# nithinp7/Pies

Hardware: AMD Instinct MI355X
Metric: substeps/sec @100k particles (PBD distance+tet-strain, 20 iterations) (higher is better)
Workload: dtype f32; 1 GPU; BASELINE configs[1]: 20x20x250 lattice beam, 100000 particles, 649156 distance + 539334 tet-strain constraints, PBD, 20 iterations, 1 substep/tick, collisions off, one body per GPU; schedule=layered, parallelism=replicas x1

## Files before the change

### include/pies_hip.h

```cpp
#ifndef PIES_HIP_H
#define PIES_HIP_H

#include <stdint.h>

#ifdef __cplusplus
extern "C" {
#endif

#define PIES_ABI_VERSION 4

typedef struct pies_solver pies_solver_t;

typedef struct pies_options {
  float fixedTimestepSize;
  uint32_t timeSubsteps;
  uint32_t iterations;
  uint32_t collisionStabilizationIterations;
  float collisionThresholdDistance;
  float collisionThickness;
  float gravity;
  float damping;
  float friction;
  float staticFrictionThreshold;
  float floorHeight;
// ... 17 lines not shown
  PIES_DISTANCE = 1,
  PIES_TET = 2,
  PIES_VOLUME = 3,
  PIES_BEND = 4,
  PIES_SHAPE = 5,
  PIES_GOAL = 6,
  PIES_TRIANGLES = 7,
  PIES_LINES = 8,
  PIES_NODES = 9,
  PIES_SYSTEM_NNZ = 10,
  PIES_REST_SETS = 11,
  PIES_ROW_STENCILS = 12,
  PIES_PD_TILES = 13,
  PIES_PD_TILE_RECORDS = 14,
  PIES_PD_CG_SINGLE = 15,
  PIES_PD_WINDOW_ENTRIES = 16,
  PIES_PD_WINDOW_HALO = 17,
  PIES_NODE_PAIRS = 18,
  PIES_NODES_RENUMBERED = 19,
  PIES_NODE_CONTACTS = 20,
  PIES_SKINS = 21,
  PIES_SKIN_VERTICES = 22,
  PIES_LAYER_REST_SETS = 23,
  PIES_LAYER_MAX_TILES = 24
};

enum { PIES_SCHEDULE_EXACT = 0, PIES_SCHEDULE_COLOURED = 1, PIES_SCHEDULE_LAYERED = 2 };
#define PIES_SCHEDULE_DEFAULT PIES_SCHEDULE_LAYERED

enum {
  PIES_FLAG_RELEASE_HINGE = 0,
  PIES_FLAG_NODE_COLLISIONS = 1,
  PIES_FLAG_TRIANGLE_COLLISIONS = 2,
  PIES_FLAG_REFERENCE_COLLISION_ORDER = 3,
  PIES_FLAG_COLLISION_ORDER = 4,
  PIES_FLAG_RENUMBER_NODES = 5,
  PIES_FLAG_PD_NODE_CONTACTS = 6
};
enum { PIES_COLLISION_ORDER_REFERENCE = 0, PIES_COLLISION_ORDER_GROUPS = 1, PIES_COLLISION_ORDER_PAIRS = 2 };

enum { PIES_NODE_POSITION = 0, PIES_NODE_PREV_POSITION = 1, PIES_NODE_VELOCITY = 2, PIES_NODE_RADIUS = 3, PIES_NODE_INV_MASS = 4 };

#define PIES_DEVICE_NONE (-1)
int pies_create(const pies_options_t* options, int device, pies_solver_t** out);
int pies_destroy(pies_solver_t* s);
int pies_clear(pies_solver_t* s);
const char* pies_last_error(const pies_solver_t* s);
// ... 106 lines not shown
```

### pies_amd/capi.py

```python
import ctypes as C
import os

import numpy as np

HERE = os.path.dirname(os.path.abspath(__file__))
LIB_PATH = os.environ.get("PIES_LIB") or os.path.join(HERE, "lib", "libpies_hip.so")

OK, ERR_INVALID, ERR_HIP, ERR_STATE, ERR_UNSUPPORTED = range(5)
PBD, PD = 0, 1
POSITION, DISTANCE, TET, VOLUME, BEND, SHAPE, GOAL, TRIANGLES, LINES, NODES = range(10)
SCHEDULE_EXACT, SCHEDULE_COLOURED, SCHEDULE_LAYERED = 0, 1, 2
SCHEDULE_DEFAULT = SCHEDULE_LAYERED
DEVICE_NONE = -1
FLAG_RELEASE_HINGE, FLAG_NODE_COLLISIONS, FLAG_TRIANGLE_COLLISIONS, FLAG_REFERENCE_COLLISION_ORDER, FLAG_COLLISION_ORDER = 0, 1, 2, 3, 4
FLAG_RENUMBER_NODES = 5
FLAG_PD_NODE_CONTACTS = 6
COLLISION_ORDER_REFERENCE, COLLISION_ORDER_GROUPS, COLLISION_ORDER_PAIRS = 0, 1, 2
NODE_POSITION, NODE_PREV_POSITION, NODE_VELOCITY, NODE_RADIUS, NODE_INV_MASS = range(5)
KERNEL_NAMES = ["predict", "position", "distance", "tet", "bend", "floor", "velocity", "hash", "collide",
                "pd_predict", "pd_local_distance", "pd_local_tet", "pd_local_volume", "pd_rhs", "pd_spmv", "pd_cg_update",
                "pd_velocity", "wave", "layer"]
KERNEL_PREDICT, KERNEL_POSITION, KERNEL_DISTANCE, KERNEL_TET, KERNEL_BEND, KERNEL_FLOOR, KERNEL_VELOCITY = range(7)
KERNEL_COUNT = 19
SYSTEM_NNZ = 10
REST_SETS = 11
ROW_STENCILS = 12
PD_TILES = 13
PD_TILE_RECORDS = 14
PD_CG_SINGLE = 15
PD_WINDOW_ENTRIES, PD_WINDOW_HALO = 16, 17
NODE_PAIRS = 18
NODES_RENUMBERED = 19
NODE_CONTACTS = 20
SKINS, SKIN_VERTICES = 21, 22
LAYER_REST_SETS = 23
LAYER_MAX_TILES = 24
LAYER_REST_MAX_SETS = 64

SYMBOLS = [
    "pies_create", "pies_destroy", "pies_clear", "pies_last_error", "pies_abi_version", "pies_default_options",
    "pies_get_options", "pies_add_nodes", "pies_add_nodes_ex", "pies_add_position_constraints",
    "pies_add_distance_constraints", "pies_add_tet_constraints", "pies_add_volume_constraints",
    "pies_add_bend_constraints", "pies_add_triangles", "pies_create_tet_box", "pies_create_box", "pies_create_sheet",
    "pies_create_bend_sheet", "pies_set_flag", "pies_set_schedule", "pies_finalize", "pies_tick", "pies_tick_async",
    "pies_synchronize", "pies_failed", "pies_count", "pies_read_nodes", "pies_write_nodes", "pies_get_ids",
    "pies_get_rest", "pies_get_order", "pies_get_batches", "pies_profile_substep", "pies_launch_counts",
    "pies_set_pcg", "pies_get_pcg_stats", "pies_collision_pairs", "pies_add_shape_constraint",
    "pies_add_goal_constraint", "pies_set_goal_transform", "pies_add_fixed_regions", "pies_update_fixed_regions",
    "pies_add_linked_regions", "pies_create_shape_matching_box", "pies_create_shape_matching_sheet", "pies_get_group",
    "pies_get_tri_contacts", "pies_tick_begin", "pies_export_acquire", "pies_export_release",
    "pies_read_positions_strided", "pies_set_pcg_retry", "pies_get_pcg_health", "pies_profile_in_situ",
    "pies_collision_stats", "pies_get_collision_health", "pies_set_collision_rounds", "pies_set_solver", "pies_debug_pair_state", "pies_set_tuning",
    "pies_get_pd_tile_plan", "pies_get_tri_grid_stats", "pies_set_rest", "pies_get_collision_fallbacks",
    "pies_add_node_pair_constraints", "pies_get_node_order", "pies_get_node_contacts",
    "pies_add_skin", "pies_get_skin_binding", "pies_read_skin", "pies_export_acquire_skin",
    "pies_voxelize_tri_mesh", "pies_add_tri_mesh_volume",
    "pies_layer_rest_pack", "pies_layer_rest_unpack", "pies_layer_rest_usable",
]

# ... 567 lines not shown
```

### pies_amd/csrc/capi.cpp

```cpp
#include <algorithm>
#include <cmath>
#include <cstdio>
#include <cstdlib>
#include <cstring>

#include "capi_internal.h"
#include "layer_rest.h"

#include <numeric>

using namespace pies;

extern "C" {

int pies_abi_version(void) { return PIES_ABI_VERSION; }

void pies_default_options(pies_options_t* o) {
  if (!o) return;
  o->fixedTimestepSize = 0.012f;
  o->timeSubsteps = 1;
  o->iterations = 4;
  o->collisionStabilizationIterations = 4;
  o->collisionThresholdDistance = 0.1f;
  o->collisionThickness = 0.05f;
// ... 694 lines not shown
    case PIES_BEND: *out = (uint32_t)s->h_bend.size(); break;
    case PIES_NODE_PAIRS: *out = (uint32_t)s->h_nodePair.size(); break;
    case PIES_SHAPE: *out = (uint32_t)s->h_shape.size(); break;
    case PIES_GOAL: *out = (uint32_t)s->h_goal.size(); break;
    case PIES_TRIANGLES: *out = (uint32_t)(s->h_triangles.size() / 3); break;
    case PIES_LINES: *out = (uint32_t)s->h_lines.size(); break;
    case PIES_NODES: *out = s->nodeCount(); break;
    case PIES_SYSTEM_NNZ: *out = s->pd_nnz; break;
    case PIES_REST_SETS: *out = s->pdLocalPacked && s->dev.d_pairDictIndex ? s->dev.pairDictSets : 0u; break;
    case PIES_ROW_STENCILS: *out = s->dev.pd.cg.rowStencil ? s->dev.pdRowStencils : 0u; break;
    case PIES_PD_TILES: *out = s->dev.pd.tiles.ntiles; break;
    case PIES_PD_TILE_RECORDS: *out = s->dev.pd.tiles.ntiles ? s->pdTileRecords : 0u; break;
    case PIES_PD_CG_SINGLE: *out = s->opt.solver == PIES_SOLVER_PD && pd_single_cg(s) ? 1u : 0u; break;
    case PIES_PD_WINDOW_ENTRIES: *out = s->dev.pd.cg.wRows ? s->pdWindowEntries : 0u; break;
    case PIES_PD_WINDOW_HALO: *out = s->dev.pd.cg.wRows ? s->pdWindowHalo : 0u; break;
    case PIES_NODES_RENUMBERED: *out = s->nodeOrder.active() ? 1u : 0u; break;
    case PIES_LAYER_REST_SETS: *out = s->layer.active ? s->layer.restSets : 0u; break;
    case PIES_LAYER_MAX_TILES: {
      *out = 0;
      if (s->layer.active)
        for (int ph = 0; ph < 4; ++ph) *out = std::max<uint32_t>(*out, (uint32_t)s->layer.tiles[ph].size());
      break;
    }
    case PIES_SKINS: *out = (uint32_t)s->h_skins.size(); break;
    case PIES_SKIN_VERTICES: {
      *out = 0;
      for (const HostSkin& k : s->h_skins) *out += k.vertexCount();
      break;
    }
    case PIES_NODE_CONTACTS: {
      *out = 0;
      if (s->device != PIES_DEVICE_NONE && s->dev.ncActive && s->dev.nd.n)
        if (int rc = nc_download(const_cast<pies_solver*>(s), nullptr, out)) return rc;
      break;
    }
    default: return PIES_ERR_INVALID;
  }
  return PIES_OK;
}

int pies_read_nodes(pies_solver_t* s, int what, float* out, uint32_t n) {
  if (!s || (!out && n)) return PIES_ERR_INVALID;
  if (n != s->nodeCount()) return fail(s, PIES_ERR_INVALID, "pies_read_nodes: n does not match the node count");
  if (s->device != PIES_DEVICE_NONE && what >= PIES_NODE_POSITION && what <= PIES_NODE_VELOCITY) {
    HIP_TRY(s, hipSetDevice(s->device));
    if (int rc = download_nodes(s, 1u << what)) return rc;
// ... 164 lines not shown
```

### pies_amd/csrc/dev_math.h

```cpp
#pragma once
#include <hip/hip_runtime.h>

namespace pies {

#define PIES_DEV __device__ __forceinline__

#ifdef PIES_BOUNDS
static __device__ unsigned int g_pies_bounds[2];
PIES_DEV bool pies_bounds_note(bool ok, unsigned int site) {
  if (!ok) {
    atomicCAS(&g_pies_bounds[0], 0u, site);
    atomicAdd(&g_pies_bounds[1], 1u);
  }
  return ok;
}
#define PIES_IN_BOUNDS(cond, site) (::pies::pies_bounds_note((cond), (site)))
#define PIES_CLAMP_INDEX(i, n) ((i) < (n) ? (i) : 0u)
#define PIES_BOUNDS_REPORT(name)                                                                                     \
  extern "C" int pies_exp_bounds_##name(unsigned int* out) {                                                         \
    unsigned int zero[2] = {0u, 0u};                                                                                 \
    if (hipMemcpyFromSymbol(out, HIP_SYMBOL(::pies::g_pies_bounds), sizeof(zero)) != hipSuccess) return 1;           \
    return hipMemcpyToSymbol(HIP_SYMBOL(::pies::g_pies_bounds), zero, sizeof(zero)) == hipSuccess ? 0 : 1;           \
  }
#else
#define PIES_IN_BOUNDS(cond, site) (true)
#define PIES_CLAMP_INDEX(i, n) (i)
#define PIES_BOUNDS_REPORT(name)
#endif

PIES_DEV uint32_t xcd_block(uint32_t bid, uint32_t nwg) {
  const uint32_t q = nwg >> 3, r = nwg & 7u, x = bid & 7u;
  return (x < r ? x * (q + 1u) : r * (q + 1u) + (x - r) * q) + (bid >> 3);
}

#ifndef PIES_SVD_MAX_SWEEPS
#define PIES_SVD_MAX_SWEEPS 8
#endif
constexpr int kSvdMaxSweeps = PIES_SVD_MAX_SWEEPS;
constexpr float kSvdTol = 4.76837158203125e-07f;
constexpr float kSvdTol2 = kSvdTol * kSvdTol;
constexpr float kSvdTiny = 1.0e-18f;
constexpr float kSvdTiny2 = 1.0e-36f;

struct Svd3 {
  float b[3][3];
  float v[3][3];
  float s[3];
  float rs[3];
};

// ... 131 lines not shown
    const float c00 = fmaf(m11, m22, -(s12 * s12)), c11 = fmaf(m00, m22, -(s02 * s02)), c22 = fmaf(m00, m11, -(s01 * s01));
    const float c01 = fmaf(s02, s12, -(s01 * m22)), c02 = fmaf(s01, s12, -(s02 * m11)), c12 = fmaf(s01, s02, -(s12 * m00));
    const float a0 = fabsf(c00), a1 = fabsf(c11), a2 = fabsf(c22);
    const bool k0 = a0 >= a1 && a0 >= a2, k1 = !k0 && a1 >= a2;
    const float v0 = k0 ? c00 : (k1 ? c01 : c02), v1 = k0 ? c01 : (k1 ? c11 : c12), v2 = k0 ? c02 : (k1 ? c12 : c22);
    const float n2 = fmaf(v2, v2, fmaf(v1, v1, v0 * v0));
    const bool okn = n2 > kSvdTiny2;
    const float in = rsqrt_nr(okn ? n2 : 1.0f);
    const float nx = okn ? v0 * in : 0.0f, ny = okn ? v1 * in : 0.0f, nz = okn ? v2 * in : 1.0f;
    const float sg = __builtin_copysignf(1.0f, nz);
    const float aa = -recip12(fabsf(nz) + 1.0f) * sg;
    const float bb = (nx * ny) * aa;
    const float V[3][3] = {{fmaf(sg * nx, nx * aa, 1.0f), sg * bb, -(sg * nx)}, {bb, fmaf(ny, ny * aa, sg), -ny}, {nx, ny, nz}};
#pragma unroll
    for (int i = 0; i < 3; ++i)
#pragma unroll
      for (int k = 0; k < 3; ++k) {
        d.v[i][k] = V[i][k];
        d.b[i][k] = fmaf(A[2][k], V[i][2], fmaf(A[1][k], V[i][1], A[0][k] * V[i][0]));
      }
    (void)jacobi_pair<0, 1>(d);
    jacobi_polish(d);
  } else {
#pragma unroll
    for (int i = 0; i < 3; ++i)
#pragma unroll
      for (int k = 0; k < 3; ++k) {
        d.b[i][k] = A[i][k];
        d.v[i][k] = (i == k) ? 1.0f : 0.0f;
      }
    if (n01) jacobi_rotate<0, 1>(d, s00, s11, s01);
    else if (n02) jacobi_rotate<0, 2>(d, s00, s22, s02);
    else if (n12) jacobi_rotate<1, 2>(d, s11, s22, s12);
  }
  float n0 = s00, n1 = s11, n2 = s22;
  if (cnt != 0) {
    bool clean = false;
    for (int sweep = 0; sweep < kSvdMaxSweeps; ++sweep) {
      n0 = dot3f(d.b[0], d.b[0]); n1 = dot3f(d.b[1], d.b[1]); n2 = dot3f(d.b[2], d.b[2]);
      const float g02 = dot3f(d.b[0], d.b[2]), g12 = dot3f(d.b[1], d.b[2]), g01 = dot3f(d.b[0], d.b[1]);
      const bool t02 = pair_needs(n0, n2, g02), t12 = pair_needs(n1, n2, g12), t01 = pair_needs(n0, n1, g01);
      clean = !(int(t02) | int(t12) | int(t01));
      if (clean) break;
      (void)jacobi_pair<0, 2>(d);
      (void)jacobi_pair<1, 2>(d);
      (void)jacobi_pair<0, 1>(d);
    }
    if (!clean) { n0 = dot3f(d.b[0], d.b[0]); n1 = dot3f(d.b[1], d.b[1]); n2 = dot3f(d.b[2], d.b[2]); }
  }
  const float nn[3] = {n0, n1, n2};
#pragma unroll
  for (int i = 0; i < 3; ++i) {
    const bool ok = nn[i] > kSvdTiny2;
    const float r = rsqrt_nr(ok ? nn[i] : 1.0f);
    d.rs[i] = ok ? r : 0.0f;
    d.s[i] = nn[i] * d.rs[i];
  }
}

template <int K, int I, int J> PIES_DEV void complete_t(const Svd3& d, float t[3][3], float sg) {
  float ui[3], uj[3];
#pragma unroll
  for (int c = 0; c < 3; ++c) {
    ui[c] = d.b[I][c] * d.rs[I];
    uj[c] = d.b[J][c] * d.rs[J];
  }
  t[K][0] = sg * (ui[1] * uj[2] - ui[2] * uj[1]);
  t[K][1] = sg * (ui[2] * uj[0] - ui[0] * uj[2]);
  t[K][2] = sg * (ui[0] * uj[1] - ui[1] * uj[0]);
}

PIES_DEV void svd3_recompose(const Svd3& d, const float snew[3], float out[3][3]) {
  float t[3][3];
  const bool ok0 = d.s[0] > kSvdTiny, ok1 = d.s[1] > kSvdTiny, ok2 = d.s[2] > kSvdTiny;
  const float g0 = ok0 ? snew[0] * d.rs[0] : 0.0f;
  const float g1 = ok1 ? snew[1] * d.rs[1] : 0.0f;
  const float g2 = ok2 ? snew[2] * d.rs[2] : 0.0f;
#pragma unroll
  for (int k = 0; k < 3; ++k) {
    t[0][k] = d.b[0][k] * g0;
    t[1][k] = d.b[1][k] * g1;
    t[2][k] = d.b[2][k] * g2;
  }
  const int nbad = (ok0 ? 0 : 1) + (ok1 ? 0 : 1) + (ok2 ? 0 : 1);
  if (nbad == 1) {
    if (!ok0) complete_t<0, 1, 2>(d, t, snew[0]);
    else if (!ok1) complete_t<1, 2, 0>(d, t, snew[1]);
    else complete_t<2, 0, 1>(d, t, snew[2]);
  }
#pragma unroll
  for (int r = 0; r < 3; ++r)
#pragma unroll
    for (int c = 0; c < 3; ++c) out[r][c] = fmaf(t[2][r], d.v[2][c], fmaf(t[1][r], d.v[1][c], t[0][r] * d.v[0][c]));
}

PIES_DEV float clampf(float v, float lo, float hi) { return fminf(fmaxf(v, lo), hi); }

PIES_DEV void mat3_mul_cm(const float p[3][3], const float q[3][3], float f[3][3]) {
#pragma unroll
  for (int c = 0; c < 3; ++c)
#pragma unroll
    for (int r = 0; r < 3; ++r) f[c][r] = p[0][r] * q[c][0] + p[1][r] * q[c][1] + p[2][r] * q[c][2];
}

PIES_DEV float det3_cm(const float m[3][3]) {
  return +m[0][0] * (m[1][1] * m[2][2] - m[2][1] * m[1][2]) - m[1][0] * (m[0][1] * m[2][2] - m[2][1] * m[0][2]) +
         m[2][0] * (m[0][1] * m[1][2] - m[1][1] * m[0][2]);
}
// ... 3 lines not shown
```

### pies_amd/csrc/layer_kernels.hip

```cpp
#include <cstdlib>

#include "dev_math.h"
#include "kernels.h"
#include "layer_rest.h"
#include "pbd_project.h"

namespace pies {

constexpr uint32_t kOffStride = kLayerMaxCols + 2;

PIES_DEV void lds_barrier() { asm volatile("s_waitcnt lgkmcnt(0)\n\ts_barrier" ::: "memory"); }
constexpr int kDistPreloadMax = 12;
constexpr int kBatch = 4;

#ifdef PIES_EXPERIMENTS
__device__ unsigned long long* g_layer_stamps = nullptr;
constexpr int kStampsPerTile = 128;
#define PIES_STAMP_DECL unsigned long long* stampBase = nullptr; int stampIdx = 0; \
  if (g_layer_stamps && tid == 0) stampBase = g_layer_stamps + (static_cast<size_t>(L.stampSlot) * 4096u + g) * kStampsPerTile;
#define PIES_STAMP() do { if (stampBase && stampIdx < kStampsPerTile) stampBase[stampIdx++] = __builtin_amdgcn_s_memtime(); } while (0)
#define PIES_STAMP_REAL() do { if (stampBase && stampIdx < kStampsPerTile) stampBase[stampIdx++] = __builtin_amdgcn_s_memrealtime(); } while (0)
#else
#define PIES_STAMP_DECL
#define PIES_STAMP()
#define PIES_STAMP_REAL()
#endif

PIES_DEV uint32_t lo16(uint32_t v) { return v & 0xFFFFu; }
PIES_DEV uint32_t hi16(uint32_t v) { return v >> 16; }

template <int BLOCK, int TETV, int WPE = 1, bool DICT = false>
__global__ void __launch_bounds__(BLOCK, WPE) k_layer(NodeArrays nd, LayerData D, LayerLaunch L, LayerParams P) {
  static_assert(3 * kLayerRestMaxSets <= BLOCK, "the prologue requests the rest dictionary with one load per lane");
  constexpr int kDistPreload = (WPE > 1 || BLOCK > 512) ? 6 : kDistPreloadMax;
  constexpr int kDistAhead = 3;
  extern __shared__ float4 lds[];
  float4* __restrict__ sp = lds;
  float4* __restrict__ stab = sp + D.maxGroupNodes;
  const uint32_t tabLen = DICT ? 3u * D.restSets : 0u;
  float* __restrict__ srad = reinterpret_cast<float*>(stab + tabLen);
  uint32_t* __restrict__ soff = reinterpret_cast<uint32_t*>(srad + D.maxGroupNodes);
  const uint32_t tid = threadIdx.x;
  const uint32_t g = xcd_block(blockIdx.x, L.groups);
  const uint4 tile = L.tileList[g];
  const uint32_t m = tile.y + tile.w;
  if (m == 0) return;
  if (!PIES_IN_BOUNDS(m <= D.maxGroupNodes, 10u)) return;
  PIES_STAMP_DECL
  PIES_STAMP_REAL();
  PIES_STAMP();
  auto lp = [&](uint32_t i) { return i < tile.y ? tile.x + i : tile.z + (i - tile.y); };

  const bool needRadius = L.needRadius != 0;
  uint32_t segCols[kLayerMaxSegs];
// ... 60 lines not shown
    for (uint32_t i = kBatch * BLOCK + tid; i < m; i += BLOCK) srad[i] = D.lrad[lp(i)];
  }
#pragma unroll
  for (int s = 0; s < kLayerMaxSegs; ++s) {
    const uint32_t nc = segCols[s];
    if (nc != 0) {
      if (tid <= nc + 1) soff[s * kOffStride + tid] = offReg[s];
      for (uint32_t c = tid + BLOCK; c <= nc + 1; c += BLOCK) soff[s * kOffStride + c] = (segOff[s] + static_cast<size_t>(g) * (nc + 1))[min(c, nc)];
    }
  }
  if (DICT && tid < tabLen) stab[tid] = tabReg;
  __syncthreads();
  PIES_STAMP();

  auto tet_ids = [&](const uint2& w, uint32_t& i1, uint32_t& i2, uint32_t& i3, uint32_t& i4) {
    if (DICT) { i1 = w.x & kLayerRestIdMask; i2 = (w.x >> 16) & kLayerRestIdMask; i3 = w.y & kLayerRestIdMask; i4 = (w.y >> 16) & kLayerRestIdMask; }
    else { i1 = lo16(w.x); i2 = hi16(w.x); i3 = lo16(w.y); i4 = hi16(w.y); }
  };
  auto rest_ok = [&](const uint2& w) { return !DICT || PIES_IN_BOUNDS(layer_rest_set(w.x, w.y) < D.restSets, 14u); };
  auto rest_read = [&](const uint2& w, float4& q0, float4& q1, float4& q2) {
    const float4* __restrict__ row = stab + 3u * layer_rest_set(w.x, w.y);
    q0 = row[0]; q1 = row[1]; q2 = row[2];
  };

  for (uint32_t s = 0; s < L.nseg; ++s) {
    const uint32_t kind = L.seg[s].kind, ncol = L.seg[s].ncol;
    const uint32_t* __restrict__ off = soff + s * kOffStride;
    if (kind == LAYER_TET && (WPE > 1 || BLOCK > 512)) {
      for (uint32_t c = 0; c < ncol; ++c) {
        for (uint32_t t = off[c] + tid; t < off[c + 1]; t += BLOCK) {
          const uint2 jd = D.tc_lid[t];
          uint32_t i1, i2, i3, i4;
          tet_ids(jd, i1, i2, i3, i4);
          if (!rest_ok(jd)) continue;
          float4 q0, q1, q2;
          if (DICT) rest_read(jd, q0, q1, q2);
          else { q0 = D.tc_q0[t]; q1 = D.tc_q1[t]; q2 = D.tc_q2[t]; }
          float4 x1 = sp[i1], x2 = sp[i2], x3 = sp[i3], x4 = sp[i4];
          tet_core<TETV>(x1, x2, x3, x4, q0, q1, q2);
          sp[i1] = x1; sp[i2] = x2; sp[i3] = x3; sp[i4] = x4;
        }
        lds_barrier();
      }
    } else if (kind == LAYER_TET) {
      const uint32_t last = off[ncol] > off[0] ? off[ncol] - 1 : 0;
      uint32_t lo = off[0], hi = off[1];
      bool have = lo + tid < hi;
      uint32_t t0 = min(lo + tid, last);
      uint2 id = D.tc_lid[t0];
      float4 a0, a1, a2, b0, b1, b2;
      if (!DICT) { a0 = D.tc_q0[t0]; a1 = D.tc_q1[t0]; a2 = D.tc_q2[t0]; }
      for (uint32_t c = 0; c < ncol; ++c) {
        const uint32_t nlo = hi, nhi = off[c + 2];
        const bool nhave = nlo + tid < nhi;
        t0 = min(nlo + tid, last);
        const uint2 nid = D.tc_lid[t0];
        if (!DICT) { b0 = D.tc_q0[t0]; b1 = D.tc_q1[t0]; b2 = D.tc_q2[t0]; }
        uint32_t i1, i2, i3, i4;
        tet_ids(id, i1, i2, i3, i4);
        if (have && PIES_IN_BOUNDS(max(max(i1, i2), max(i3, i4)) < m, 11u) && rest_ok(id)) {
          if (DICT) rest_read(id, a0, a1, a2);
          float4 x1 = sp[i1], x2 = sp[i2], x3 = sp[i3], x4 = sp[i4];
#ifdef PIES_EXPERIMENTS
          if (stampBase) { asm volatile("s_waitcnt lgkmcnt(0)" ::: "memory"); PIES_STAMP(); }
#endif
          tet_core<TETV>(x1, x2, x3, x4, a0, a1, a2);
#ifdef PIES_EXPERIMENTS
          if (stampBase) { asm volatile("" : "+v"(x1.x), "+v"(x2.x), "+v"(x3.x), "+v"(x4.x)); PIES_STAMP(); }
#endif
          sp[i1] = x1; sp[i2] = x2; sp[i3] = x3; sp[i4] = x4;
        }
        for (uint32_t t = lo + tid + BLOCK; t < hi; t += BLOCK) {
          const uint2 jd = D.tc_lid[t];
          uint32_t j1, j2, j3, j4;
          tet_ids(jd, j1, j2, j3, j4);
          if (!rest_ok(jd)) continue;
          float4 q0, q1, q2;
          if (DICT) rest_read(jd, q0, q1, q2);
          else { q0 = D.tc_q0[t]; q1 = D.tc_q1[t]; q2 = D.tc_q2[t]; }
          float4 x1 = sp[j1], x2 = sp[j2], x3 = sp[j3], x4 = sp[j4];
          tet_core<TETV>(x1, x2, x3, x4, q0, q1, q2);
          sp[j1] = x1; sp[j2] = x2; sp[j3] = x3; sp[j4] = x4;
        }
        lds_barrier();
        PIES_STAMP();
        lo = nlo; hi = nhi; have = nhave; id = nid;
        if (!DICT) { a0 = b0; a1 = b1; a2 = b2; }
      }
    } else if (kind == LAYER_DISTANCE) {
      const uint32_t last = off[ncol] > off[0] ? off[ncol] - 1 : 0;
      uint32_t id[kDistPreload];
      float2 rw[kDistPreload];
#pragma unroll
      for (int c = 0; c < kDistPreload; ++c) { id[c] = 0u; rw[c] = make_float2(0.f, 0.f); }
#pragma unroll
      for (int c = 0; c < kDistAhead; ++c) {
        const uint32_t cc = min(static_cast<uint32_t>(c), ncol - 1);
        const uint32_t t = min(off[cc] + tid, last);
        id[c] = D.dc_lid[t];
        rw[c] = D.dc_rw[t];
      }
#pragma unroll
      for (int c = 0; c < kDistPreload; ++c) {
        if (static_cast<uint32_t>(c) < ncol) {
// ... 166 lines not shown
  if (nd.n == 0) return;
  if (toNodeArray) hipLaunchKernelGGL(k_lcopy<true>, node_grid(nd.n), dim3(kNodeBlock), 0, st, nd.pos, D.nodeList, D.lpos, nd.n);
  else hipLaunchKernelGGL(k_lcopy<false>, node_grid(nd.n), dim3(kNodeBlock), 0, st, nd.pos, D.nodeList, D.lpos, nd.n);
}

#ifdef PIES_EXPERIMENTS
extern "C" int pies_exp_layer_stamps(unsigned long long* deviceBuffer) {
  return hipMemcpyToSymbol(HIP_SYMBOL(g_layer_stamps), &deviceBuffer, sizeof(deviceBuffer)) == hipSuccess ? 0 : 1;
}
#endif
PIES_BOUNDS_REPORT(layer)
size_t layer_lds_bytes(uint32_t maxGroupNodes, uint32_t restSets) {
  return static_cast<size_t>(maxGroupNodes) * (sizeof(float4) + sizeof(float)) + kLayerMaxSegs * kOffStride * sizeof(uint32_t) +
         static_cast<size_t>(restSets) * 3u * sizeof(float4);
}

template <bool DICT>
static hipError_t layer_prepare_variants(int bytes) {
  hipError_t e = hipFuncSetAttribute(reinterpret_cast<const void*>(k_layer<256, 0, 1, DICT>), hipFuncAttributeMaxDynamicSharedMemorySize, bytes);
  if (e == hipSuccess) e = hipFuncSetAttribute(reinterpret_cast<const void*>(k_layer<512, 0, 1, DICT>), hipFuncAttributeMaxDynamicSharedMemorySize, bytes);
  if (e == hipSuccess) e = hipFuncSetAttribute(reinterpret_cast<const void*>(k_layer<512, 0, 4, DICT>), hipFuncAttributeMaxDynamicSharedMemorySize, bytes);
  if (e == hipSuccess) e = hipFuncSetAttribute(reinterpret_cast<const void*>(k_layer<256, 0, 4, DICT>), hipFuncAttributeMaxDynamicSharedMemorySize, bytes);
  if (e == hipSuccess) e = hipFuncSetAttribute(reinterpret_cast<const void*>(k_layer<1024, 0, 1, DICT>), hipFuncAttributeMaxDynamicSharedMemorySize, bytes);
  return e;
}
hipError_t layer_prepare(uint32_t maxGroupNodes, uint32_t restSets) {
  const int bytes = static_cast<int>(layer_lds_bytes(maxGroupNodes, restSets));
  if (bytes <= 64 * 1024) return hipSuccess;
  return restSets ? layer_prepare_variants<true>(bytes) : layer_prepare_variants<false>(bytes);
}

template <bool DICT>
static void launch_layer_variant(hipStream_t st, uint32_t want, bool throughput, size_t lds, const NodeArrays& nd, const LayerData& D,
                                 const LayerLaunch& L, const LayerParams& P) {
  if (want <= 256 && throughput) hipLaunchKernelGGL((k_layer<256, 0, 4, DICT>), dim3(L.groups), dim3(256), lds, st, nd, D, L, P);
  else if (want <= 256) hipLaunchKernelGGL((k_layer<256, 0, 1, DICT>), dim3(L.groups), dim3(256), lds, st, nd, D, L, P);
  else if (want <= 512 && throughput) hipLaunchKernelGGL((k_layer<512, 0, 4, DICT>), dim3(L.groups), dim3(512), lds, st, nd, D, L, P);
  else if (want <= 512) hipLaunchKernelGGL((k_layer<512, 0, 1, DICT>), dim3(L.groups), dim3(512), lds, st, nd, D, L, P);
  else hipLaunchKernelGGL((k_layer<1024, 0, 1, DICT>), dim3(L.groups), dim3(1024), lds, st, nd, D, L, P);
}

void launch_layer(hipStream_t st, const NodeArrays& nd, const LayerData& D, const LayerLaunch& L0, const LayerParams& P) {
  if (L0.groups == 0 || L0.nseg == 0) return;
  LayerLaunch L = L0;
  L.tileList = D.tiles[L.phase];
  for (uint32_t s = L.nseg; s < static_cast<uint32_t>(kLayerMaxSegs); ++s) L.seg[s] = LayerSeg{};
  L.needRadius = 0u;
  for (uint32_t s = 0; s < L.nseg; ++s) L.needRadius |= (L.seg[s].kind == LAYER_FLOOR || L.seg[s].kind == LAYER_VELOCITY) ? 1u : 0u;
  const bool restDict = D.tc_rest && D.restSets && D.restSets <= kLayerRestMaxSets;
  const size_t lds = layer_lds_bytes(D.maxGroupNodes, restDict ? D.restSets : 0u);
#ifdef PIES_EXPERIMENTS
  const int skipMask = [] { const char* e = getenv("PIES_EXP_LAYER_SKIP"); return e ? atoi(e) : 0; }();
  if (skipMask) {
    L.nseg = 0;
    for (uint32_t s = 0; s < L0.nseg; ++s)
      if (!((skipMask >> L0.seg[s].kind) & 1)) L.seg[L.nseg++] = L0.seg[s];
  }
  {
    static unsigned int slot = 0;
    L.stampSlot = slot++ & 63u;
  }
  const int variant = [] { const char* e = getenv("PIES_EXP_TET"); return e ? atoi(e) : 0; }();
  if (variant == 1) {
    if (restDict) hipLaunchKernelGGL((k_layer<256, 1, 1, true>), dim3(L.groups), dim3(256), lds, st, nd, D, L, P);
    else hipLaunchKernelGGL((k_layer<256, 1>), dim3(L.groups), dim3(256), lds, st, nd, D, L, P);
    return;
  }
#endif
  const uint32_t forceBlock = [] { const char* e = tuning_env("PIES_LAYER_BLOCK"); return e ? (uint32_t)atoi(e) : 0u; }();
  uint32_t want = forceBlock ? forceBlock : L.maxClass;
  if (!forceBlock && L.groups > 256u) want = std::min<uint32_t>(want, 512u);
  const bool throughput = L.groups > 256u;
  if (restDict) launch_layer_variant<true>(st, want, throughput, lds, nd, D, L, P);
  else launch_layer_variant<false>(st, want, throughput, lds, nd, D, L, P);
}

}
```

Before: 907.1 substeps/s.

## Add packed-pair row-form tet strain projection variant for layered kernel

Adds a new tet-strain projection (tet_rows.h) that packs two of the three column components into float2 vectors so the compiler can emit packed FP32 ops. It uses wave-uniform ballot guards around the rare SVD fallback paths. It also reads dictionary rest data directly from LDS inside the projection. The variant is selected by default for non-throughput launches with at most 512 threads. Intended to cut VALU instruction count in the SVD/polar step, at the risk of numeric differences and higher register pressure.

```diff
diff --git a/include/pies_hip.h b/include/pies_hip.h
--- a/include/pies_hip.h
+++ b/include/pies_hip.h
@@ -63,7 +63,8 @@
   PIES_SKINS = 21,
   PIES_SKIN_VERTICES = 22,
   PIES_LAYER_REST_SETS = 23,
-  PIES_LAYER_MAX_TILES = 24
+  PIES_LAYER_MAX_TILES = 24,
+  PIES_LAYER_MAX_CLASS = 25
 };
 
 enum { PIES_SCHEDULE_EXACT = 0, PIES_SCHEDULE_COLOURED = 1, PIES_SCHEDULE_LAYERED = 2 };
diff --git a/pies_amd/capi.py b/pies_amd/capi.py
--- a/pies_amd/capi.py
+++ b/pies_amd/capi.py
@@ -35,6 +35,7 @@
 SKINS, SKIN_VERTICES = 21, 22
 LAYER_REST_SETS = 23
 LAYER_MAX_TILES = 24
+LAYER_MAX_CLASS = 25
 LAYER_REST_MAX_SETS = 64
 
 SYMBOLS = [
diff --git a/pies_amd/csrc/capi.cpp b/pies_amd/csrc/capi.cpp
--- a/pies_amd/csrc/capi.cpp
+++ b/pies_amd/csrc/capi.cpp
@@ -740,6 +740,12 @@
         for (int ph = 0; ph < 4; ++ph) *out = std::max<uint32_t>(*out, (uint32_t)s->layer.tiles[ph].size());
       break;
     }
+    case PIES_LAYER_MAX_CLASS: {
+      *out = 0;
+      if (s->layer.active)
+        for (const LayerKind& K : s->layer.kind) *out = std::max<uint32_t>(*out, K.maxClass);
+      break;
+    }
     case PIES_SKINS: *out = (uint32_t)s->h_skins.size(); break;
     case PIES_SKIN_VERTICES: {
       *out = 0;
diff --git a/pies_amd/csrc/dev_math.h b/pies_amd/csrc/dev_math.h
--- a/pies_amd/csrc/dev_math.h
+++ b/pies_amd/csrc/dev_math.h
@@ -26,6 +26,14 @@
 #define PIES_IN_BOUNDS(cond, site) (true)
 #define PIES_CLAMP_INDEX(i, n) (i)
 #define PIES_BOUNDS_REPORT(name)
+#endif
+
+#ifdef PIES_PATH_NOTES
+#define PIES_RARE_PATH() asm volatile("; pies-rare-path")
+#define PIES_MAIN_TET_PATH() asm volatile("; pies-main-tet-path")
+#else
+#define PIES_RARE_PATH()
+#define PIES_MAIN_TET_PATH()
 #endif
 
 PIES_DEV uint32_t xcd_block(uint32_t bid, uint32_t nwg) {
@@ -203,6 +211,7 @@
     (void)jacobi_pair<0, 1>(d);
     jacobi_polish(d);
   } else {
+    PIES_RARE_PATH();
 #pragma unroll
     for (int i = 0; i < 3; ++i)
 #pragma unroll
@@ -223,6 +232,7 @@
       const bool t02 = pair_needs(n0, n2, g02), t12 = pair_needs(n1, n2, g12), t01 = pair_needs(n0, n1, g01);
       clean = !(int(t02) | int(t12) | int(t01));
       if (clean) break;
+      PIES_RARE_PATH();
       (void)jacobi_pair<0, 2>(d);
       (void)jacobi_pair<1, 2>(d);
       (void)jacobi_pair<0, 1>(d);
@@ -265,6 +275,7 @@
   }
   const int nbad = (ok0 ? 0 : 1) + (ok1 ? 0 : 1) + (ok2 ? 0 : 1);
   if (nbad == 1) {
+    PIES_RARE_PATH();
     if (!ok0) complete_t<0, 1, 2>(d, t, snew[0]);
     else if (!ok1) complete_t<1, 2, 0>(d, t, snew[1]);
     else complete_t<2, 0, 1>(d, t, snew[2]);
diff --git a/pies_amd/csrc/layer_kernels.hip b/pies_amd/csrc/layer_kernels.hip
--- a/pies_amd/csrc/layer_kernels.hip
+++ b/pies_amd/csrc/layer_kernels.hip
@@ -4,6 +4,7 @@
 #include "kernels.h"
 #include "layer_rest.h"
 #include "pbd_project.h"
+#include "tet_rows.h"
 
 namespace pies {
 
@@ -29,7 +30,7 @@
 PIES_DEV uint32_t lo16(uint32_t v) { return v & 0xFFFFu; }
 PIES_DEV uint32_t hi16(uint32_t v) { return v >> 16; }
 
-template <int BLOCK, int TETV, int WPE = 1, bool DICT = false>
+template <int BLOCK, int TETV, int WPE = 1, bool DICT = false, int FORM = 0>
 __global__ void __launch_bounds__(BLOCK, WPE) k_layer(NodeArrays nd, LayerData D, LayerLaunch L, LayerParams P) {
   static_assert(3 * kLayerRestMaxSets <= BLOCK, "the prologue requests the rest dictionary with one load per lane");
   constexpr int kDistPreload = (WPE > 1 || BLOCK > 512) ? 6 : kDistPreloadMax;
@@ -136,6 +137,15 @@
     const float4* __restrict__ row = stab + 3u * layer_rest_set(w.x, w.y);
     q0 = row[0]; q1 = row[1]; q2 = row[2];
   };
+  auto project = [&](const uint2& w, float4& x1, float4& x2, float4& x3, float4& x4, float4& q0, float4& q1, float4& q2) {
+    if (FORM == 1 && TETV == 0) {
+      if (DICT) rows::tet_rows(x1, x2, x3, x4, rows::rest_of(reinterpret_cast<const float*>(stab + 3u * layer_rest_set(w.x, w.y))));
+      else rows::tet_rows(x1, x2, x3, x4, rows::rest_of(q0, q1, q2));
+    } else {
+      if (DICT) rest_read(w, q0, q1, q2);
+      tet_core<TETV>(x1, x2, x3, x4, q0, q1, q2);
+    }
+  };
 
   for (uint32_t s = 0; s < L.nseg; ++s) {
     const uint32_t kind = L.seg[s].kind, ncol = L.seg[s].ncol;
@@ -173,27 +183,27 @@
         uint32_t i1, i2, i3, i4;
         tet_ids(id, i1, i2, i3, i4);
         if (have && PIES_IN_BOUNDS(max(max(i1, i2), max(i3, i4)) < m, 11u) && rest_ok(id)) {
-          if (DICT) rest_read(id, a0, a1, a2);
+          PIES_MAIN_TET_PATH();
           float4 x1 = sp[i1], x2 = sp[i2], x3 = sp[i3], x4 = sp[i4];
 #ifdef PIES_EXPERIMENTS
           if (stampBase) { asm volatile("s_waitcnt lgkmcnt(0)" ::: "memory"); PIES_STAMP(); }
 #endif
-          tet_core<TETV>(x1, x2, x3, x4, a0, a1, a2);
+          project(id, x1, x2, x3, x4, a0, a1, a2);
 #ifdef PIES_EXPERIMENTS
           if (stampBase) { asm volatile("" : "+v"(x1.x), "+v"(x2.x), "+v"(x3.x), "+v"(x4.x)); PIES_STAMP(); }
 #endif
           sp[i1] = x1; sp[i2] = x2; sp[i3] = x3; sp[i4] = x4;
         }
         for (uint32_t t = lo + tid + BLOCK; t < hi; t += BLOCK) {
+          PIES_RARE_PATH();
           const uint2 jd = D.tc_lid[t];
           uint32_t j1, j2, j3, j4;
           tet_ids(jd, j1, j2, j3, j4);
           if (!rest_ok(jd)) continue;
           float4 q0, q1, q2;
-          if (DICT) rest_read(jd, q0, q1, q2);
-          else { q0 = D.tc_q0[t]; q1 = D.tc_q1[t]; q2 = D.tc_q2[t]; }
+          if (!DICT) { q0 = D.tc_q0[t]; q1 = D.tc_q1[t]; q2 = D.tc_q2[t]; }
           float4 x1 = sp[j1], x2 = sp[j2], x3 = sp[j3], x4 = sp[j4];
-          tet_core<TETV>(x1, x2, x3, x4, q0, q1, q2);
+          project(jd, x1, x2, x3, x4, q0, q1, q2);
           sp[j1] = x1; sp[j2] = x2; sp[j3] = x3; sp[j4] = x4;
         }
         lds_barrier();
@@ -406,6 +416,8 @@
   if (e == hipSuccess) e = hipFuncSetAttribute(reinterpret_cast<const void*>(k_layer<512, 0, 4, DICT>), hipFuncAttributeMaxDynamicSharedMemorySize, bytes);
   if (e == hipSuccess) e = hipFuncSetAttribute(reinterpret_cast<const void*>(k_layer<256, 0, 4, DICT>), hipFuncAttributeMaxDynamicSharedMemorySize, bytes);
   if (e == hipSuccess) e = hipFuncSetAttribute(reinterpret_cast<const void*>(k_layer<1024, 0, 1, DICT>), hipFuncAttributeMaxDynamicSharedMemorySize, bytes);
+  if (e == hipSuccess) e = hipFuncSetAttribute(reinterpret_cast<const void*>(k_layer<256, 0, 1, DICT, 1>), hipFuncAttributeMaxDynamicSharedMemorySize, bytes);
+  if (e == hipSuccess) e = hipFuncSetAttribute(reinterpret_cast<const void*>(k_layer<512, 0, 1, DICT, 1>), hipFuncAttributeMaxDynamicSharedMemorySize, bytes);
   return e;
 }
 hipError_t layer_prepare(uint32_t maxGroupNodes, uint32_t restSets) {
@@ -415,8 +427,13 @@
 }
 
 template <bool DICT>
-static void launch_layer_variant(hipStream_t st, uint32_t want, bool throughput, size_t lds, const NodeArrays& nd, const LayerData& D,
-                                 const LayerLaunch& L, const LayerParams& P) {
+static void launch_layer_variant(hipStream_t st, uint32_t want, bool throughput, bool rowForm, size_t lds, const NodeArrays& nd,
+                                 const LayerData& D, const LayerLaunch& L, const LayerParams& P) {
+  if (rowForm && !throughput && want <= 512) {
+    if (want <= 256) hipLaunchKernelGGL((k_layer<256, 0, 1, DICT, 1>), dim3(L.groups), dim3(256), lds, st, nd, D, L, P);
+    else hipLaunchKernelGGL((k_layer<512, 0, 1, DICT, 1>), dim3(L.groups), dim3(512), lds, st, nd, D, L, P);
+    return;
+  }
   if (want <= 256 && throughput) hipLaunchKernelGGL((k_layer<256, 0, 4, DICT>), dim3(L.groups), dim3(256), lds, st, nd, D, L, P);
   else if (want <= 256) hipLaunchKernelGGL((k_layer<256, 0, 1, DICT>), dim3(L.groups), dim3(256), lds, st, nd, D, L, P);
   else if (want <= 512 && throughput) hipLaunchKernelGGL((k_layer<512, 0, 4, DICT>), dim3(L.groups), dim3(512), lds, st, nd, D, L, P);
@@ -455,8 +472,9 @@
   uint32_t want = forceBlock ? forceBlock : L.maxClass;
   if (!forceBlock && L.groups > 256u) want = std::min<uint32_t>(want, 512u);
   const bool throughput = L.groups > 256u;
-  if (restDict) launch_layer_variant<true>(st, want, throughput, lds, nd, D, L, P);
-  else launch_layer_variant<false>(st, want, throughput, lds, nd, D, L, P);
-}
-
-}
+  const bool rowForm = [] { const char* e = tuning_env("PIES_LAYER_TET_FORM"); return !e || e[0] != '0'; }();
+  if (restDict) launch_layer_variant<true>(st, want, throughput, rowForm, lds, nd, D, L, P);
+  else launch_layer_variant<false>(st, want, throughput, rowForm, lds, nd, D, L, P);
+}
+
+}
diff --git a/pies_amd/csrc/tet_rows.h b/pies_amd/csrc/tet_rows.h
--- /dev/null
+++ b/pies_amd/csrc/tet_rows.h
@@ -0,0 +1,358 @@
+#pragma once
+#if defined(__HIP__)
+#include "dev_math.h"
+#define PIES_ROWS_FN __device__ __forceinline__
+#define PIES_ROWS_UNROLL _Pragma("unroll")
+#else
+#include <cmath>
+#include <cstdint>
+#include <cstring>
+#define PIES_ROWS_FN inline
+#define PIES_ROWS_UNROLL
+#define PIES_RARE_PATH()
+#endif
+
+namespace pies {
+namespace rows {
+
+#if defined(__HIP__)
+PIES_ROWS_FN float rf_fma(float a, float b, float c) { return fmaf(a, b, c); }
+PIES_ROWS_FN float rf_abs(float a) { return fabsf(a); }
+PIES_ROWS_FN float rf_min(float a, float b) { return fminf(a, b); }
+PIES_ROWS_FN float rf_max(float a, float b) { return fmaxf(a, b); }
+PIES_ROWS_FN float rf_copysign(float a, float b) { return __builtin_copysignf(a, b); }
+PIES_ROWS_FN int rf_bits(float a) { return __float_as_int(a); }
+PIES_ROWS_FN float rf_float(int a) { return __int_as_float(a); }
+PIES_ROWS_FN bool any_lane(bool p) { return __builtin_amdgcn_ballot_w64(p) != 0ull; }
+#else
+inline float rf_fma(float a, float b, float c) { return std::fmaf(a, b, c); }
+inline float rf_abs(float a) { return std::fabs(a); }
+inline float rf_min(float a, float b) { return std::fmin(a, b); }
+inline float rf_max(float a, float b) { return std::fmax(a, b); }
+inline float rf_copysign(float a, float b) { return std::copysign(a, b); }
+inline int rf_bits(float a) { int32_t i; std::memcpy(&i, &a, 4); return i; }
+inline float rf_float(int a) { float f; std::memcpy(&f, &a, 4); return f; }
+inline bool any_lane(bool p) { return p; }
+#endif
+
+#if defined(__HIP__) && !defined(PIES_ROWS_SCALAR)
+typedef float rp __attribute__((ext_vector_type(2)));
+PIES_ROWS_FN rp rp_make(float x, float y) { return rp{x, y}; }
+PIES_ROWS_FN rp rp_add(rp a, rp b) { return a + b; }
+PIES_ROWS_FN rp rp_sub(rp a, rp b) { return a - b; }
+PIES_ROWS_FN rp rp_mul(rp a, rp b) { return a * b; }
+PIES_ROWS_FN rp rp_neg(rp a) { return -a; }
+PIES_ROWS_FN rp rp_fma(rp a, rp b, rp c) { return __builtin_elementwise_fma(a, b, c); }
+#else
+struct rp {
+  float x, y;
+};
+PIES_ROWS_FN rp rp_make(float x, float y) { return rp{x, y}; }
+PIES_ROWS_FN rp rp_add(rp a, rp b) { return rp{a.x + b.x, a.y + b.y}; }
+PIES_ROWS_FN rp rp_sub(rp a, rp b) { return rp{a.x - b.x, a.y - b.y}; }
+PIES_ROWS_FN rp rp_mul(rp a, rp b) { return rp{a.x * b.x, a.y * b.y}; }
+PIES_ROWS_FN rp rp_neg(rp a) { return rp{-a.x, -a.y}; }
+PIES_ROWS_FN rp rp_fma(rp a, rp b, rp c) { return rp{rf_fma(a.x, b.x, c.x), rf_fma(a.y, b.y, c.y)}; }
+#endif
+PIES_ROWS_FN rp rp_splat(float a) { return rp_make(a, a); }
+
+struct Col {
+  rp p;
+  float z;
+};
+
+constexpr int kMaxSweeps = 8;
+constexpr float kTol = 4.76837158203125e-07f;
+constexpr float kTol2 = kTol * kTol;
+constexpr float kTiny = 1.0e-18f;
+constexpr float kTiny2 = 1.0e-36f;
+constexpr float kCos[8] = {8.660253882e-01f,  1.666651964e-01f, -4.807964712e-02f, 2.440584078e-02f,
+                           -1.432729699e-02f, 7.718813606e-03f, -2.961986931e-03f, 5.536798271e-04f};
+#if defined(__HIP__)
+static_assert(kMaxSweeps == kSvdMaxSweeps && kTol == kSvdTol && kTiny == kSvdTiny && kTiny2 == kSvdTiny2 && kCos[0] == kCos3[0] &&
+                  kCos[1] == kCos3[1] && kCos[2] == kCos3[2] && kCos[3] == kCos3[3] && kCos[4] == kCos3[4] && kCos[5] == kCos3[5] &&
+                  kCos[6] == kCos3[6] && kCos[7] == kCos3[7],
+              "tet_rows.h restates dev_math.h's constants");
+#endif
+
+PIES_ROWS_FN float rsqrt_nr(float x) {
+  float y = rf_float(0x5f3759df - (rf_bits(x) >> 1));
+  const float hx = 0.5f * x;
+  y = y * rf_fma(-hx, y * y, 1.5f);
+  y = y * rf_fma(-hx, y * y, 1.5f);
+  y = y * rf_fma(-hx, y * y, 1.5f);
+  return y;
+}
+PIES_ROWS_FN float recip12(float t) {
+  float y = rf_fma(-0.47058824f, t, 1.4117647f);
+  y = y * rf_fma(-t, y, 2.0f);
+  y = y * rf_fma(-t, y, 2.0f);
+  y = y * rf_fma(-t, y, 2.0f);
+  return y;
+}
+PIES_ROWS_FN float recip_rough(float x) {
+  float y = rf_float(0x7EF311C7 - (rf_bits(x) & 0x7fffffff));
+  y = y * rf_fma(-rf_abs(x), y, 2.0f);
+  y = y * rf_fma(-rf_abs(x), y, 2.0f);
+  return rf_copysign(y, x);
+}
+PIES_ROWS_FN float cdot(const Col& a, const Col& b) { return rf_fma(a.z, b.z, rf_fma(a.p.y, b.p.y, a.p.x * b.p.x)); }
+PIES_ROWS_FN bool pair_needs(float alpha, float beta, float gamma) { return gamma * gamma > rf_fma(kTol2, alpha * beta, kTiny2); }
+
+template <int P, int Q> PIES_ROWS_FN void rotate(Col (&b)[3], Col (&v)[3], const float alpha, const float beta, const float gamma) {
+  const float delta = beta - alpha;
+  const float g2 = gamma + gamma;
+  const float hw = rf_fma(delta, delta, g2 * g2);
+  const float h = hw * rsqrt_nr(hw);
+  const float c1 = h + rf_abs(delta);
+  const float s1 = delta < 0.0f ? -g2 : g2;
+  const float inv = rsqrt_nr(rf_fma(c1, c1, s1 * s1));
+  const float cs = c1 * inv, sn = s1 * inv;
+  const rp cs2 = rp_splat(cs), sn2 = rp_splat(sn);
+  const Col x = b[P], y = b[Q], vx = v[P], vy = v[Q];
+  b[P].p = rp_fma(cs2, x.p, rp_neg(rp_mul(sn2, y.p)));
+  b[P].z = rf_fma(cs, x.z, -(sn * y.z));
+  b[Q].p = rp_fma(sn2, x.p, rp_mul(cs2, y.p));
+  b[Q].z = rf_fma(sn, x.z, cs * y.z);
+  v[P].p = rp_fma(cs2, vx.p, rp_neg(rp_mul(sn2, vy.p)));
+  v[P].z = rf_fma(cs, vx.z, -(sn * vy.z));
+  v[Q].p = rp_fma(sn2, vx.p, rp_mul(cs2, vy.p));
+  v[Q].z = rf_fma(sn, vx.z, cs * vy.z);
+}
+template <int P, int Q> PIES_ROWS_FN void test_pair(Col (&b)[3], Col (&v)[3]) {
+  const float alpha = cdot(b[P], b[P]);
+  const float beta = cdot(b[Q], b[Q]);
+  const float gamma = cdot(b[P], b[Q]);
+  const bool need = pair_needs(alpha, beta, gamma);
+  if (!any_lane(need)) return;
+  if (need) rotate<P, Q>(b, v, alpha, beta, gamma);
+}
+PIES_ROWS_FN void polish(Col (&b)[3], Col (&v)[3], bool* guarded = nullptr) {
+  const float n0 = cdot(b[0], b[0]), n1 = cdot(b[1], b[1]), n2 = cdot(b[2], b[2]);
+  const float g01 = cdot(b[0], b[1]), g02 = cdot(b[0], b[2]), g12 = cdot(b[1], b[2]);
+  float t01 = g01 * recip_rough(n1 - n0), t02 = g02 * recip_rough(n2 - n0), t12 = g12 * recip_rough(n2 - n1);
+  if (guarded) *guarded = !(rf_abs(t01) <= 3.0e38f) || !(rf_abs(t02) <= 3.0e38f) || !(rf_abs(t12) <= 3.0e38f);
+  if (!(rf_abs(t01) < 2.5e-4f)) t01 = 0.0f;
+  if (!(rf_abs(t02) < 2.5e-4f)) t02 = 0.0f;
+  if (!(rf_abs(t12) < 2.5e-4f)) t12 = 0.0f;
+  const rp p01 = rp_splat(t01), p02 = rp_splat(t02), p12 = rp_splat(t12);
+  const rp m01 = rp_splat(-t01), m02 = rp_splat(-t02), m12 = rp_splat(-t12);
+  const Col x = b[0], y = b[1], z = b[2];
+  b[0].p = rp_fma(m02, z.p, rp_fma(m01, y.p, x.p));
+  b[0].z = rf_fma(-t02, z.z, rf_fma(-t01, y.z, x.z));
+  b[1].p = rp_fma(m12, z.p, rp_fma(p01, x.p, y.p));
+  b[1].z = rf_fma(-t12, z.z, rf_fma(t01, x.z, y.z));
+  b[2].p = rp_fma(p12, y.p, rp_fma(p02, x.p, z.p));
+  b[2].z = rf_fma(t12, y.z, rf_fma(t02, x.z, z.z));
+  const Col vx = v[0], vy = v[1], vz = v[2];
+  v[0].p = rp_fma(m02, vz.p, rp_fma(m01, vy.p, vx.p));
+  v[0].z = rf_fma(-t02, vz.z, rf_fma(-t01, vy.z, vx.z));
+  v[1].p = rp_fma(m12, vz.p, rp_fma(p01, vx.p, vy.p));
+  v[1].z = rf_fma(-t12, vz.z, rf_fma(t01, vx.z, vy.z));
+  v[2].p = rp_fma(p12, vy.p, rp_fma(p02, vx.p, vz.p));
+  v[2].z = rf_fma(t12, vy.z, rf_fma(t02, vx.z, vz.z));
+}
+
+struct Paths {
+  bool closedForm = false, identity = false, onePair = false, rangeOut = false, fallback = false, exhausted = false;
+  bool completed = false, twoCollapsed = false, flipped = false, polishGuard = false;
+  int sweeps = 0;
+};
+
+PIES_ROWS_FN void svd(const Col (&a)[3], Col (&b)[3], Col (&v)[3], float (&s)[3], float (&rs)[3], Paths* paths) {
+  const float s00 = cdot(a[0], a[0]), s11 = cdot(a[1], a[1]), s22 = cdot(a[2], a[2]);
+  const float s01 = cdot(a[0], a[1]), s02 = cdot(a[0], a[2]), s12 = cdot(a[1], a[2]);
+  const bool n01 = pair_needs(s00, s11, s01), n02 = pair_needs(s00, s22, s02), n12 = pair_needs(s11, s22, s12);
+  const int cnt = (n01 ? 1 : 0) + (n02 ? 1 : 0) + (n12 ? 1 : 0);
+  const float q = ((s00 + s11) + s22) * 0.333333343f;
+  const float d0 = s00 - q, d1 = s11 - q, d2 = s22 - q;
+  const float p1 = rf_fma(s12, s12, rf_fma(s02, s02, s01 * s01));
+  const float p2 = rf_fma(d0, d0, rf_fma(d1, d1, rf_fma(d2, d2, p1 + p1)));
+  const bool closed = cnt >= 2 && p2 > 1.0e-30f && p2 < 1.0e16f;
+  if (closed) {
+    const float w = p2 * 0.166666672f;
+    const float ip = rsqrt_nr(w);
+    const float p = w * ip;
+    const float det = rf_fma(d0, rf_fma(d1, d2, -(s12 * s12)), rf_fma(s02, rf_fma(s01, s12, -(d1 * s02)), -(s01 * rf_fma(s01, d2, -(s12 * s02)))));
+    const float r = ((0.5f * det) * ip) * (ip * ip);
+    const float x = rf_min(rf_abs(r), 1.0f);
+    float c = kCos[7];
+PIES_ROWS_UNROLL
+    for (int k = 6; k >= 0; --k) c = rf_fma(c, x, kCos[k]);
+    const float lam = q + rf_copysign((p + p) * c, r);
+    const float m00 = s00 - lam, m11 = s11 - lam, m22 = s22 - lam;
+    const float c00 = rf_fma(m11, m22, -(s12 * s12)), c11 = rf_fma(m00, m22, -(s02 * s02)), c22 = rf_fma(m00, m11, -(s01 * s01));
+    const float c01 = rf_fma(s02, s12, -(s01 * m22)), c02 = rf_fma(s01, s12, -(s02 * m11)), c12 = rf_fma(s01, s02, -(s12 * m00));
+    const float a0 = rf_abs(c00), a1 = rf_abs(c11), a2 = rf_abs(c22);
+    const bool k0 = a0 >= a1 && a0 >= a2, k1 = !k0 && a1 >= a2;
+    const float v0 = k0 ? c00 : (k1 ? c01 : c02), v1 = k0 ? c01 : (k1 ? c11 : c12), v2 = k0 ? c02 : (k1 ? c12 : c22);
+    const float n2 = rf_fma(v2, v2, rf_fma(v1, v1, v0 * v0));
+    const bool okn = n2 > kTiny2;
+    const float in = rsqrt_nr(okn ? n2 : 1.0f);
+    const float nx = okn ? v0 * in : 0.0f, ny = okn ? v1 * in : 0.0f, nz = okn ? v2 * in : 1.0f;
+    const float sg = rf_copysign(1.0f, nz);
+    const float aa = -recip12(rf_abs(nz) + 1.0f) * sg;
+    const float bb = (nx * ny) * aa;
+    v[0].p = rp_make(rf_fma(sg * nx, nx * aa, 1.0f), sg * bb);
+    v[0].z = -(sg * nx);
+    v[1].p = rp_make(bb, rf_fma(ny, ny * aa, sg));
+    v[1].z = -ny;
+    v[2].p = rp_make(nx, ny);
+    v[2].z = nz;
+PIES_ROWS_UNROLL
+    for (int i = 0; i < 3; ++i) {
+      const float vi0 = v[i].p.x, vi1 = v[i].p.y, vi2 = v[i].z;
+      b[i].p = rp_fma(a[2].p, rp_splat(vi2), rp_fma(a[1].p, rp_splat(vi1), rp_mul(a[0].p, rp_splat(vi0))));
+      b[i].z = rf_fma(a[2].z, vi2, rf_fma(a[1].z, vi1, a[0].z * vi0));
+    }
+    test_pair<0, 1>(b, v);
+    polish(b, v, paths ? &paths->polishGuard : nullptr);
+  }
+  if (any_lane(!closed)) {
+    if (!closed) {
+      PIES_RARE_PATH();
+PIES_ROWS_UNROLL
+      for (int i = 0; i < 3; ++i) {
+        b[i] = a[i];
+        v[i].p = rp_make(i == 0 ? 1.0f : 0.0f, i == 1 ? 1.0f : 0.0f);
+        v[i].z = i == 2 ? 1.0f : 0.0f;
+      }
+      if (n01) rotate<0, 1>(b, v, s00, s11, s01);
+      else if (n02) rotate<0, 2>(b, v, s00, s22, s02);
+      else if (n12) rotate<1, 2>(b, v, s11, s22, s12);
+    }
+  }
+  float n0 = cdot(b[0], b[0]), n1 = cdot(b[1], b[1]), n2 = cdot(b[2], b[2]);
+  bool clean;
+  {
+    const float g02 = cdot(b[0], b[2]), g12 = cdot(b[1], b[2]), g01 = cdot(b[0], b[1]);
+    const bool t02 = pair_needs(n0, n2, g02), t12 = pair_needs(n1, n2, g12), t01 = pair_needs(n0, n1, g01);
+    clean = !(int(t02) | int(t12) | int(t01));
+  }
+  if (any_lane(!clean)) {
+    if (!clean) {
+      PIES_RARE_PATH();
+      for (int sweep = 1;; ++sweep) {
+        test_pair<0, 2>(b, v);
+        test_pair<1, 2>(b, v);
+        test_pair<0, 1>(b, v);
+        n0 = cdot(b[0], b[0]); n1 = cdot(b[1], b[1]); n2 = cdot(b[2], b[2]);
+        if (sweep == kMaxSweeps) break;
+        const float g02 = cdot(b[0], b[2]), g12 = cdot(b[1], b[2]), g01 = cdot(b[0], b[1]);
+        const bool t02 = pair_needs(n0, n2, g02), t12 = pair_needs(n1, n2, g12), t01 = pair_needs(n0, n1, g01);
+        clean = !(int(t02) | int(t12) | int(t01));
+        if (paths) paths->sweeps = sweep;
+        if (clean) break;
+      }
+      if (paths) { paths->fallback = true; paths->exhausted = !clean; }
+    }
+  }
+  if (paths) {
+    paths->closedForm = closed;
+    paths->identity = cnt == 0;
+    paths->onePair = cnt == 1;
+    paths->rangeOut = cnt >= 2 && !closed;
+  }
+  const float nn[3] = {n0, n1, n2};
+PIES_ROWS_UNROLL
+  for (int i = 0; i < 3; ++i) {
+    const bool ok = nn[i] > kTiny2;
+    const float r = rsqrt_nr(ok ? nn[i] : 1.0f);
+    rs[i] = ok ? r : 0.0f;
+    s[i] = nn[i] * rs[i];
+  }
+}
+
+template <int K, int I, int J> PIES_ROWS_FN void complete(const Col (&b)[3], const float (&rs)[3], Col (&t)[3], const float sg) {
+  const float ui0 = b[I].p.x * rs[I], ui1 = b[I].p.y * rs[I], ui2 = b[I].z * rs[I];
+  const float uj0 = b[J].p.x * rs[J], uj1 = b[J].p.y * rs[J], uj2 = b[J].z * rs[J];
+  t[K].p = rp_make(sg * (ui1 * uj2 - ui2 * uj1), sg * (ui2 * uj0 - ui0 * uj2));
+  t[K].z = sg * (ui0 * uj1 - ui1 * uj0);
+}
+
+PIES_ROWS_FN void recompose(const Col (&b)[3], const Col (&v)[3], const float (&s)[3], const float (&rs)[3], const float (&snew)[3],
+                            Col (&out)[3], Paths* paths) {
+  const bool ok0 = s[0] > kTiny, ok1 = s[1] > kTiny, ok2 = s[2] > kTiny;
+  const float g0 = ok0 ? snew[0] * rs[0] : 0.0f;
+  const float g1 = ok1 ? snew[1] * rs[1] : 0.0f;
+  const float g2 = ok2 ? snew[2] * rs[2] : 0.0f;
+  Col t[3];
+  t[0].p = rp_mul(b[0].p, rp_splat(g0)); t[0].z = b[0].z * g0;
+  t[1].p = rp_mul(b[1].p, rp_splat(g1)); t[1].z = b[1].z * g1;
+  t[2].p = rp_mul(b[2].p, rp_splat(g2)); t[2].z = b[2].z * g2;
+  const int nbad = (ok0 ? 0 : 1) + (ok1 ? 0 : 1) + (ok2 ? 0 : 1);
+  if (any_lane(nbad == 1)) {
+    if (nbad == 1) {
+      PIES_RARE_PATH();
+      if (!ok0) complete<0, 1, 2>(b, rs, t, snew[0]);
+      else if (!ok1) complete<1, 2, 0>(b, rs, t, snew[1]);
+      else complete<2, 0, 1>(b, rs, t, snew[2]);
+    }
+  }
+  if (paths) { paths->completed = nbad == 1; paths->twoCollapsed = nbad >= 2; }
+  out[0].p = rp_fma(rp_splat(t[2].p.x), v[2].p, rp_fma(rp_splat(t[1].p.x), v[1].p, rp_mul(rp_splat(t[0].p.x), v[0].p)));
+  out[0].z = rf_fma(t[2].p.x, v[2].z, rf_fma(t[1].p.x, v[1].z, t[0].p.x * v[0].z));
+  out[1].p = rp_fma(rp_splat(t[2].p.y), v[2].p, rp_fma(rp_splat(t[1].p.y), v[1].p, rp_mul(rp_splat(t[0].p.y), v[0].p)));
+  out[1].z = rf_fma(t[2].p.y, v[2].z, rf_fma(t[1].p.y, v[1].z, t[0].p.y * v[0].z));
+  out[2].p = rp_fma(rp_splat(t[2].z), v[2].p, rp_fma(rp_splat(t[1].z), v[1].p, rp_mul(rp_splat(t[0].z), v[0].p)));
+  out[2].z = rf_fma(t[2].z, v[2].z, rf_fma(t[1].z, v[1].z, t[0].z * v[0].z));
+}
+
+struct Rest {
+  rp q0, q1, q2;
+  float q20, q21, q22, lo, hi, w;
+};
+template <class V4> PIES_ROWS_FN Rest rest_of(const V4& a0, const V4& a1, const V4& a2) {
+  return Rest{rp_make(a0.x, a0.w), rp_make(a0.y, a1.x), rp_make(a0.z, a1.y), a1.z, a1.w, a2.x, a2.y, a2.z, a2.w};
+}
+PIES_ROWS_FN Rest rest_of(const float* __restrict__ r) {
+  return Rest{rp_make(r[0], r[3]), rp_make(r[1], r[4]), rp_make(r[2], r[5]), r[6], r[7], r[8], r[9], r[10], r[11]};
+}
+
+template <class V4> PIES_ROWS_FN void tet_rows(V4& x1, V4& x2, V4& x3, V4& x4, const Rest& R, Paths* paths = nullptr) {
+  const float e0[3] = {x2.x - x1.x, x3.x - x1.x, x4.x - x1.x};
+  const float e1[3] = {x2.y - x1.y, x3.y - x1.y, x4.y - x1.y};
+  const float e2[3] = {x2.z - x1.z, x3.z - x1.z, x4.z - x1.z};
+  Col A[3];
+  A[0].p = rp_add(rp_add(rp_mul(rp_splat(e0[0]), R.q0), rp_mul(rp_splat(e0[1]), R.q1)), rp_mul(rp_splat(e0[2]), R.q2));
+  A[0].z = e0[0] * R.q20 + e0[1] * R.q21 + e0[2] * R.q22;
+  A[1].p = rp_add(rp_add(rp_mul(rp_splat(e1[0]), R.q0), rp_mul(rp_splat(e1[1]), R.q1)), rp_mul(rp_splat(e1[2]), R.q2));
+  A[1].z = e1[0] * R.q20 + e1[1] * R.q21 + e1[2] * R.q22;
+  A[2].p = rp_add(rp_add(rp_mul(rp_splat(e2[0]), R.q0), rp_mul(rp_splat(e2[1]), R.q1)), rp_mul(rp_splat(e2[2]), R.q2));
+  A[2].z = e2[0] * R.q20 + e2[1] * R.q21 + e2[2] * R.q22;
+  const float f00 = A[0].p.x, f10 = A[0].p.y, f20 = A[0].z, f01 = A[1].p.x, f11 = A[1].p.y, f21 = A[1].z, f02 = A[2].p.x, f12 = A[2].p.y,
+              f22 = A[2].z;
+  const float detF = +f00 * (f11 * f22 - f21 * f12) - f10 * (f01 * f22 - f21 * f02) + f20 * (f01 * f12 - f11 * f02);
+  Col B[3], V[3];
+  float s[3], rs[3];
+  svd(A, B, V, s, rs, paths);
+  float sn[3];
+PIES_ROWS_UNROLL
+  for (int i = 0; i < 3; ++i) sn[i] = rf_min(rf_max(s[i], R.lo), R.hi);
+  if (detF < 0.0f) {
+    int k = 0;
+    float m = s[0];
+    if (s[1] <= m) { k = 1; m = s[1]; }
+    if (s[2] <= m) { k = 2; }
+    sn[0] = (k == 0) ? -sn[0] : sn[0];
+    sn[1] = (k == 1) ? -sn[1] : sn[1];
+    sn[2] = (k == 2) ? -sn[2] : sn[2];
+  }
+  if (paths) paths->flipped = detF < 0.0f;
+  Col Fh[3];
+  recompose(B, V, s, rs, sn, Fh, paths);
+  const float w = R.w;
+  const rp w2 = rp_splat(w);
+  const rp p1 = rp_make(x1.x, x1.y), p2 = rp_make(x2.x, x2.y), p3 = rp_make(x3.x, x3.y), p4 = rp_make(x4.x, x4.y);
+  const rp r1 = rp_add(p1, rp_mul(w2, rp_sub(rp_splat(0.0f), p1)));
+  const rp r2 = rp_add(p2, rp_mul(w2, rp_sub(Fh[0].p, p2)));
+  const rp r3 = rp_add(p3, rp_mul(w2, rp_sub(Fh[1].p, p3)));
+  const rp r4 = rp_add(p4, rp_mul(w2, rp_sub(Fh[2].p, p4)));
+  x1.x = r1.x; x1.y = r1.y; x1.z += w * (0.0f - x1.z);
+  x2.x = r2.x; x2.y = r2.y; x2.z += w * (Fh[0].z - x2.z);
+  x3.x = r3.x; x3.y = r3.y; x3.z += w * (Fh[1].z - x3.z);
+  x4.x = r4.x; x4.y = r4.y; x4.z += w * (Fh[2].z - x4.z);
+}
+
+}
+}
```

Result: faster. 977.5 substeps/s (median of 6 runs) (+7.8%).
